# zixunh/vipe

Measured on AMD Instinct MI355X. Metric: dense-BA+flow update iters/s, 512x384 48-KF graph, higher is better.
Workload: dtype f16 (correlation, GRU; fp32 accumulate) + f32 geometry/BA (fp64 reduced system)

## Files before the change

include/vipe_amd.h:

```cpp
#ifndef VIPE_AMD_H
#define VIPE_AMD_H

#include <stdint.h>

#ifdef __cplusplus
extern "C" {
#endif

#define VIPE_F16 0
#define VIPE_F32 1
#define VIPE_F64 2
#define VIPE_U8 3

#define VIPE_OK 0
#define VIPE_EINVAL (-1)
#define VIPE_ENOSPACE (-2)
#define VIPE_EUNSUPPORTED (-3)

#define VIPE_PYRAMID_REFERENCE 0
#define VIPE_PYRAMID_BLOCKED 1

#define VIPE_CAM_PINHOLE 0
#define VIPE_CAM_MEI 1
#define VIPE_CAM_PANORAMA 2
// ... 200 lines not shown

int vipe_corr_sampler_forward(const void* d_in1, const void* d_in2, void* d_out, int B, int C, int H, int W, int kH,
                              int kW, int patchH, int patchW, int padH, int padW, int dilH, int dilW,
                              int dil_patchH, int dil_patchW, int dH, int dW, int dtype, void* stream);
int vipe_corr_sampler_backward(const void* d_in1, const void* d_in2, const void* d_grad_out, void* d_grad1,
                               void* d_grad2, int B, int C, int H, int W, int kH, int kW, int patchH, int patchW,
                               int padH, int padW, int dilH, int dilW, int dil_patchH, int dil_patchW, int dH,
                               int dW, int dtype, void* stream);

int vipe_corr_sampler_forward_host(const float* h_in1, const float* h_in2, float* h_out, int B, int C, int H, int W, int kH,
                                   int kW, int patchH, int patchW, int padH, int padW, int dilH, int dilW, int dil_patchH,
                                   int dil_patchW, int dH, int dW);
int vipe_corr_sampler_backward_host(const float* h_in1, const float* h_in2, const float* h_grad_out, float* h_grad1,
                                    float* h_grad2, int B, int C, int H, int W, int kH, int kW, int patchH, int patchW,
                                    int padH, int padW, int dilH, int dilW, int dil_patchH, int dil_patchW, int dH, int dW);

int vipe_nearest_neighbours(const float* d_query, int qdim, const float* d_tree, int tdim, int64_t M, int64_t N, int knn,
                            float* d_dist, int* d_idx, void* stream);

int vipe_ms_deform_attn_forward(const void* d_value, const int64_t* d_spatial_shapes, const int64_t* d_level_start_index,
                                const void* d_sampling_loc, const void* d_attn_weight, void* d_output, int64_t bs,
                                int64_t Lv, int heads, int C, int L, int64_t Lq, int P, int dtype, void* stream);
int vipe_ms_deform_attn_backward(const void* d_value, const int64_t* d_spatial_shapes, const int64_t* d_level_start_index,
                                 const void* d_sampling_loc, const void* d_attn_weight, const void* d_grad_output,
                                 void* d_grad_value, void* d_grad_sampling_loc, void* d_grad_attn_weight, int64_t bs,
                                 int64_t Lv, int heads, int C, int L, int64_t Lq, int P, int dtype, void* stream);

#define VIPE_ACT_NONE 0
#define VIPE_ACT_RELU 1
#define VIPE_ACT_SIGMOID 2
#define VIPE_ACT_TANH 3
int vipe_conv_pack_weights(const void* d_w_oihw, void* d_w_packed, int Cout, int Cin, int KH, int KW, int src_dtype,
                           void* stream);
int vipe_conv2d_nhwc_f16(const void* d_x, const void* d_w_packed, const float* d_bias, const float* d_extra,
                         void* d_y, int B, int H, int W, int Cin, int cin_total, int cin_off, int Cout,
                         int cout_total, int cout_off, int KH, int KW, int act, void* stream);

int vipe_conv_packed_dims(int Cout, int Cin, int KH, int KW, int* cout_pad, int* cin_pad, int* k_pad);

#define VIPE_CONV_PARTIAL 6
#define VIPE_CONV_HEADS_FUSED 7
#define VIPE_CONV_ACCINIT_F32 0x100
int vipe_conv2d_fused(const void* d_x0, int x0_ctot, int x0_coff, const void* d_x1, int x1_ctot, int x1_coff,
                      int split, const void* d_w_packed, const float* d_bias, const float* d_extra, int extra_stride,
                      int extra_off, void* d_y, int y_ctot, int y_coff, void* d_y2, int y2_ctot, int y2_coff,
                      const void* d_net, int net_ctot, int net_coff, const void* d_z, float* d_fout,
                      const void* d_accinit, int ai_ctot, int ai_coff, int B, int H, int W, int Cin, int Cout, int KH,
                      int KW, int act, int mode, void* stream);

int vipe_heads_fused_ok(int H, int W);
int vipe_heads_border_floats(int E, int H, int W, int64_t* n_floats);
int vipe_heads_finish(float* d_dw, const float* d_border, const float* d_bias, int E, int H, int W, void* stream);

typedef struct {
  const void *corr0_w, *corr2_w, *flow0_w, *flow2_w, *gw_w, *zr_w, *q_w, *zr_s_w, *q_s_w, *heads0_w, *heads2_w, *agg2_w, *eta_w;
  const void *zr_n_w, *zr_x_w;
  const float *corr0_b, *corr2_b, *flow0_b, *flow2_b, *gw_b, *zr_b, *q_b, *heads0_b, *heads2_b, *agg2_b, *eta_b;
  const float* glo_wT;
  const float* glo_b;
  const void *agg1_w, *heads_dw_w;
  const float *agg1_b, *heads_dw_b;
  const void* heads2_frag;
} vipe_update_weights;
typedef struct {
  int E, H, W, n_src;
  const void* levels[4];
  const float* coords;
  const int* slots;
  int h2, w2, pyramid_layout;
  const void* corr;
  const void* motn;
  const void* net;
  void* net_out;
  void* xbuf;
  const void* pgate;
  void *c1, *f1, *zb, *rnet;
  void* hbuf;
  float* dw;
  float *glo, *extra;
  const int *order, *rowptr;
  void *agg, *a2;
  float* eta;
  void* side_stream;
  float* pzr;
  int gate_state;
  float* hborder;
} vipe_update_buffers;
int vipe_update_operator(const vipe_update_weights* weights, const vipe_update_buffers* buffers, void* stream);

int vipe_update_gate_state(const vipe_update_weights* weights, const vipe_update_buffers* buffers, const void* d_net,
                           int parts, void* stream);
typedef struct {
  const vipe_update_weights* weights;
  const vipe_update_buffers* buffers;
  const void* net;
  const int* bounds;
  int n_bounds;
} vipe_gate_state_job;
int vipe_update_gate_state_piece(void* user, int piece, int n_pieces, void* stream);

int vipe_glo_context(const float* d_glo_sum, const float* d_wT, const float* d_bias, float* d_extra, int E, int hw,
                     void* stream);

typedef struct {
  const void* src;
  void* dst;
// ... 88 lines not shown
```

vipe_amd/csrc/conv_mfma.hip:

```cpp
#include <stdlib.h>

#include <type_traits>

#include "common.cuh"

namespace {

typedef _Float16 half8 __attribute__((ext_vector_type(8)));
typedef _Float16 half4 __attribute__((ext_vector_type(4)));
typedef float float16v __attribute__((ext_vector_type(16)));
typedef float float4v __attribute__((ext_vector_type(4)));

enum Epi { EPI_PLAIN = 0, EPI_GLO = 1, EPI_ZR = 2, EPI_Q = 3, EPI_HEADS = 4, EPI_ETA = 5, EPI_PARTIAL = 6, EPI_HEADS_FUSED = 7 };

struct ConvArgs {
  const half_t* x0; int x0_ctot, x0_coff;
  const half_t* x1; int x1_ctot, x1_coff;
  int split;
  const half_t* w;
  const float* bias;
  const float* extra;
  int extra_stride, extra_off;
  half_t* y; int y_ctot, y_coff;
  int B, H, W, Cin, Cin_pad, Cout, Cout_pad, KH, KW, nsteps;
// ... 1051 lines not shown
    for (int j = 0; j < 4; ++j) acc[i][j] = float4v{0.0f, 0.0f, 0.0f, 0.0f};
#pragma unroll
  for (int st = 0; st < 7; ++st) {
    half8 wf[4];
#pragma unroll
    for (int i = 0; i < 4; ++i)
      wf[i] = *reinterpret_cast<const half8*>(lds + (st >> 1) * 16384 + swz(wm * 64 + i * 16 + l16, (st & 1) * 4 + lk));
    const int t0 = min(st * 8 + lk * 2, 48), t1 = min(st * 8 + lk * 2 + 1, 48);
    const int wrow = FLAT ? wn * HALO_TW : wn * C7_PW;
    const int o0 = (wrow + (t0 / 7) * pitch + l16 + t0 % 7) * 8, o1 = (wrow + (t1 / 7) * pitch + l16 + t1 % 7) * 8;
#pragma unroll
    for (int j = 0; j < 4; ++j) {
      const half4 lo = *reinterpret_cast<const half4*>(ldsX + o0 + j * 128);
      const half4 hi = *reinterpret_cast<const half4*>(ldsX + o1 + j * 128);
      const half8 xf = {lo[0], lo[1], lo[2], lo[3], hi[0], hi[1], hi[2], hi[3]};
#pragma unroll
      for (int i = 0; i < 4; ++i) acc[i][j] = __builtin_amdgcn_mfma_f32_16x16x32_f16(wf[i], xf, acc[i][j], 0, 0, 0);
    }
  }
  __syncthreads();
  constexpr int PITCH = 136;
  half_t* stage = reinterpret_cast<half_t*>(lds);
#pragma unroll
  for (int i = 0; i < 4; ++i) {
    const int cl = wm * 64 + i * 16 + 4 * lk;
    const float4 b = *reinterpret_cast<const float4*>(a.bias + cout0 + cl);
#pragma unroll
    for (int j = 0; j < 4; ++j) {
      half4 h;
      h[0] = (half_t)act_apply(acc[i][j][0] + b.x, a.act);
      h[1] = (half_t)act_apply(acc[i][j][1] + b.y, a.act);
      h[2] = (half_t)act_apply(acc[i][j][2] + b.z, a.act);
      h[3] = (half_t)act_apply(acc[i][j][3] + b.w, a.act);
      *reinterpret_cast<half4*>(stage + (wn * 64 + j * 16 + l16) * PITCH + cl) = h;
    }
  }
  __syncthreads();
  const int ch = (tid & 15) * 8, co = cout0 + ch;
#pragma unroll
  for (int it = 0; it < 8; ++it) {
    const int pl = (tid >> 4) + 32 * it;
    const int64_t m = pix_of(pl);
    if (FLAT && m < 0) continue;
    const half8 o = *reinterpret_cast<const half8*>(stage + pl * PITCH + ch);
    half_t* dst = a.y + m * a.y_ctot + a.y_coff + co;
    if (co + 8 <= a.Cout) {
      *reinterpret_cast<half8*>(dst) = o;
    } else {
      for (int q = 0; q < 8 && co + q < a.Cout; ++q) dst[q] = o[q];
    }
  }
}

__global__ void pack_weights_kernel(const void* __restrict__ src, half_t* __restrict__ dst, int Cout, int Cin, int KH,
                                    int KW, int Cout_pad, int Cin_pad, int K_pad, int src_f32, int smallcin) {
  const int64_t total = (int64_t)K_pad * Cout_pad;
  for (int64_t i = (int64_t)blockIdx.x * blockDim.x + threadIdx.x; i < total; i += (int64_t)gridDim.x * blockDim.x) {
    const int kin = (int)(i % 64);
    const int co = (int)((i / 64) % Cout_pad);
    const int s = (int)(i / (64 * (int64_t)Cout_pad));
    const int k = s * 64 + kin;
    int tap, c;
    if (smallcin) { tap = k / 4; c = k % 4; }
    else { tap = k / Cin_pad; c = k % Cin_pad; }
    float v = 0.0f;
    if (co < Cout && c < Cin && tap < KH * KW) {
      const int64_t o = (((int64_t)co * Cin + c) * KH + tap / KW) * KW + tap % KW;
      v = src_f32 ? reinterpret_cast<const float*>(src)[o] : (float)reinterpret_cast<const half_t*>(src)[o];
    }
    dst[i] = (half_t)v;
  }
}

inline int round_up(int x, int m) { return (x + m - 1) / m * m; }

}


extern "C" {

VIPE_EXPORT int vipe_conv_packed_dims(int Cout, int Cin, int KH, int KW, int* cout_pad, int* cin_pad, int* k_pad) {
  if (Cout <= 0 || Cin <= 0 || KH <= 0 || KW <= 0) return VIPE_EINVAL;
  const int cp = Cout <= 32 ? 32 : (Cout <= 64 ? 64 : round_up(Cout, 128));
  int cinp, kp;
  if (Cin == 4) { cinp = 4; kp = round_up(KH * KW * 4, 64); }
  else { cinp = round_up(Cin, 64); kp = KH * KW * cinp; }
  if (cout_pad) *cout_pad = cp;
  if (cin_pad) *cin_pad = cinp;
  if (k_pad) *k_pad = kp;
  return VIPE_OK;
}

VIPE_EXPORT int vipe_conv_pack_weights(const void* d_w_oihw, void* d_w_packed, int Cout, int Cin, int KH, int KW,
                                       int src_dtype, void* stream) {
  VIPE_CHECK_ARG(d_w_oihw && d_w_packed);
  VIPE_CHECK_ARG(src_dtype == VIPE_F16 || src_dtype == VIPE_F32);
  int cp, cinp, kp;
  if (vipe_conv_packed_dims(Cout, Cin, KH, KW, &cp, &cinp, &kp) != VIPE_OK) return VIPE_EINVAL;
  VIPE_CHECK_ARG(Cin == 4 || Cin % 8 == 0);
  const int64_t total = (int64_t)kp * cp;
  pack_weights_kernel<<<(int)std::min<int64_t>((total + 255) / 256, 4096), 256, 0, as_stream(stream)>>>(
      d_w_oihw, (half_t*)d_w_packed, Cout, Cin, KH, KW, cp, cinp, kp, src_dtype == VIPE_F32, Cin == 4);
  return vipe_launch_status();
}

}
// ... 204 lines not shown
                                  int y_coff, void* d_y2, int y2_ctot, int y2_coff, const void* d_net, int net_ctot,
                                  int net_coff, const void* d_z, float* d_fout, const void* d_accinit, int ai_ctot,
                                  int ai_coff, int B, int H, int W, int Cin, int Cout, int KH, int KW, int act, int mode,
                                  void* stream) {
  VIPE_CHECK_ARG(d_x0 && d_w_packed && d_bias);
  VIPE_CHECK_ARG(!d_accinit || (ai_ctot % 4 == 0 && ai_coff % 4 == 0 && ai_coff + Cout <= ai_ctot));
  VIPE_CHECK_ARG(B >= 0 && H > 0 && W > 0 && Cin > 0 && Cout > 0 && (KH & 1) && (KW & 1));
  if (Cin == 4) {
    VIPE_CHECK_ARG(split >= Cin && x0_ctot % 4 == 0 && x0_coff % 4 == 0);
  } else {
    VIPE_CHECK_ARG(Cin % 8 == 0 && x0_ctot % 8 == 0 && x0_coff % 8 == 0);
    VIPE_CHECK_ARG(split >= Cin || (split % 64 == 0 && d_x1 && x1_ctot % 8 == 0 && x1_coff % 8 == 0));
  }
  const int ai_f32 = (mode & VIPE_CONV_ACCINIT_F32) != 0;
  mode &= ~VIPE_CONV_ACCINIT_F32;
  VIPE_CHECK_ARG(mode >= EPI_PLAIN && mode <= EPI_HEADS_FUSED);
  if (mode == EPI_HEADS_FUSED) {
    VIPE_CHECK_ARG(d_fout && d_net && d_y2 && Cin == 128 && Cout == 256 && KH == 3 && KW == 3 && act == VIPE_ACT_RELU &&
                   !d_extra && !d_accinit && !ai_f32 && split >= Cin);
    if (H % HALO_TH != 0 || W % HALO_TW != 0) return VIPE_EUNSUPPORTED;
  }
  if (mode == EPI_PARTIAL) VIPE_CHECK_ARG(d_fout && y_ctot % 4 == 0 && y_coff % 4 == 0 && y_coff + Cout <= y_ctot && !d_extra);
  if (mode == EPI_PLAIN) VIPE_CHECK_ARG(d_y && y_ctot % 4 == 0 && y_coff % 4 == 0);
  if (mode == EPI_GLO) VIPE_CHECK_ARG(d_net && d_fout);
  if (mode == EPI_ZR) VIPE_CHECK_ARG(d_y && d_y2 && d_net && Cout == 256);
  if (mode == EPI_Q) VIPE_CHECK_ARG(d_y && d_net && d_z && Cout == 128);
  if (mode == EPI_HEADS) VIPE_CHECK_ARG(d_fout && Cout == 4);
  if (mode == EPI_ETA) VIPE_CHECK_ARG(d_fout && Cout == 1);
  ConvArgs a = {};
  a.x0 = (const half_t*)d_x0; a.x0_ctot = x0_ctot; a.x0_coff = x0_coff;
  a.x1 = (const half_t*)(d_x1 ? d_x1 : d_x0); a.x1_ctot = d_x1 ? x1_ctot : x0_ctot; a.x1_coff = d_x1 ? x1_coff : x0_coff;
  a.split = split > Cin ? Cin : split;
  a.w = (const half_t*)d_w_packed; a.bias = d_bias; a.extra = d_extra; a.extra_stride = extra_stride; a.extra_off = extra_off;
  a.y = (half_t*)d_y; a.y_ctot = y_ctot; a.y_coff = y_coff;
  a.y2 = (half_t*)d_y2; a.y2_ctot = y2_ctot; a.y2_coff = y2_coff;
  if (mode == EPI_HEADS_FUSED) {
    a.w2 = (const half_t*)d_net; a.border = (float*)d_y2;
    d_net = nullptr; a.y2 = nullptr;
  }
  a.net = (const half_t*)d_net; a.net_ctot = net_ctot; a.net_coff = net_coff;
  a.zbuf = (const half_t*)d_z; a.fout = d_fout;
  a.accinit = (const half_t*)d_accinit; a.ai_ctot = ai_ctot; a.ai_coff = ai_coff; a.ai_f32 = ai_f32;
  a.B = B; a.H = H; a.W = W; a.Cin = Cin; a.Cout = Cout; a.KH = KH; a.KW = KW;
  a.act = act; a.epi = mode;
  return launch_conv(a, as_stream(stream));
}

VIPE_EXPORT int vipe_heads_fused_ok(int H, int W) {
  const char* v = getenv("VIPE_AMD_FUSED_HEADS");
  const bool enabled = !(v && v[0] == '0');
  return enabled && H > 0 && W > 0 && H % HALO_TH == 0 && W % HALO_TW == 0;
}

VIPE_EXPORT int vipe_heads_border_floats(int E, int H, int W, int64_t* n) {
  VIPE_CHECK_ARG(n && E >= 0 && H > 0 && W > 0 && H % HALO_TH == 0 && W % HALO_TW == 0);
  *n = (int64_t)E * (H / HALO_TH) * (W / HALO_TW) * HB_N * 4;
  return VIPE_OK;
}

VIPE_EXPORT int vipe_heads_finish(float* d_dw, const float* d_border, const float* d_bias, int E, int H, int W, void* stream) {
  VIPE_CHECK_ARG(E >= 0 && H > 0 && W > 0 && H % HALO_TH == 0 && W % HALO_TW == 0);
  if (E == 0) return VIPE_OK;
  VIPE_CHECK_ARG(d_dw && d_border && d_bias);
  const int64_t M = (int64_t)E * H * W;
  heads_finish_kernel<<<(unsigned)((M + 255) / 256), 256, 0, as_stream(stream)>>>(d_dw, d_border, d_bias, M, H, W);
  return vipe_launch_status();
}

}
```

vipe_amd/csrc/update_op.hip:

```cpp
#include "common.cuh"

namespace {

__global__ __launch_bounds__(384) void glo_gemm_kernel(const float* __restrict__ glo, const float* __restrict__ wT ,
                                                       const float* __restrict__ b, float* __restrict__ extra, float inv_hw) {
  __shared__ float g[128];
  const int e = blockIdx.x, t = threadIdx.x;
  if (t < 128) g[t] = glo[(int64_t)e * 128 + t] * inv_hw;
  __syncthreads();
  float acc = b[t];
#pragma unroll 8
  for (int k = 0; k < 128; ++k) acc = __builtin_fmaf(g[k], wT[k * 384 + t], acc);
  extra[(int64_t)e * 384 + t] = acc;
}

__global__ __launch_bounds__(256) void update_finish_kernel(const float* __restrict__ coords1, const float* __restrict__ dw,
                                                            const unsigned char* __restrict__ mask, float* __restrict__ target,
                                                            float* __restrict__ weight, const float* __restrict__ eta,
                                                            const int64_t* __restrict__ du, float* __restrict__ damping,
                                                            int64_t n_px, int64_t n_eta, int P) {
  const int64_t i = (int64_t)blockIdx.x * 256 + threadIdx.x;
  if (i < n_px) {
    const float2 c = reinterpret_cast<const float2*>(coords1)[i];
    const float4 d = reinterpret_cast<const float4*>(dw)[i];
// ... 4 lines not shown
  if (i < n_eta) damping[du[i / P] * P + i % P] = eta[i];
}

}

namespace {
hipEvent_t* operator_events() {
  static thread_local hipEvent_t ev[64][4] = {};
  int d = 0;
  (void)hipGetDevice(&d);
  hipEvent_t* e = ev[d & 63];
  for (int i = 0; i < 4; ++i)
    if (!e[i] && hipEventCreateWithFlags(&e[i], hipEventDisableTiming) != hipSuccess) return nullptr;
  return e;
}
}

extern "C" {

VIPE_EXPORT int vipe_update_operator(const vipe_update_weights* wt, const vipe_update_buffers* b, void* stream) {
  VIPE_CHECK_ARG(wt && b && b->E >= 0 && b->H > 0 && b->W > 0);
  if (b->E == 0) return VIPE_OK;
  const int E = b->E, H = b->H, W = b->W;
  hipStream_t s = as_stream(stream);
  int rc;
#define RUN(call)              \
  do {                         \
    rc = (call);               \
    if (rc != VIPE_OK) return rc; \
  } while (0)
  hipStream_t s2 = (hipStream_t)b->side_stream;
  hipEvent_t* ev = s2 ? operator_events() : nullptr;
  if (s2 && !ev) return VIPE_EINVAL;
  void* const stream2 = s2 ? b->side_stream : stream;
#define FORK(i)                                                                                              \
  do {                                                                                                       \
    if (s2 && (hipEventRecord(ev[i], s) != hipSuccess || hipStreamWaitEvent(s2, ev[i], 0) != hipSuccess)) return VIPE_EINVAL; \
  } while (0)
#define JOIN(i)                                                                                              \
  do {                                                                                                       \
    if (s2 && (hipEventRecord(ev[i], s2) != hipSuccess || hipStreamWaitEvent(s, ev[i], 0) != hipSuccess)) return VIPE_EINVAL; \
  } while (0)
  FORK(0);
  if (b->levels[0]) {
    RUN(vipe_corr_lookup_conv1x1_ex(b->levels, b->coords, wt->corr0_w, wt->corr0_b, b->c1, 128, 0, E, H, W, b->h2, b->w2, 128,
                                    VIPE_ACT_RELU, b->slots, b->pyramid_layout, stream, 0, s2 ? 1 : 0));
  } else {
    VIPE_CHECK_ARG(b->corr);
    RUN(vipe_conv2d_fused(b->corr, 200, 0, nullptr, 0, 0, 200, wt->corr0_w, wt->corr0_b, nullptr, 0, 0, b->c1, 128, 0, nullptr,
                          0, 0, nullptr, 0, 0, nullptr, nullptr, nullptr, 0, 0, E, H, W, 200, 128, 1, 1, VIPE_ACT_RELU, 0, stream));
  }
  RUN(vipe_conv2d_fused(b->c1, 128, 0, nullptr, 0, 0, 128, wt->corr2_w, wt->corr2_b, nullptr, 0, 0, b->xbuf, 320, 128, nullptr,
                        0, 0, nullptr, 0, 0, nullptr, nullptr, nullptr, 0, 0, E, H, W, 128, 128, 3, 3, VIPE_ACT_RELU, 0, stream));
  RUN(vipe_conv2d_fused(b->motn, 4, 0, nullptr, 0, 0, 4, wt->flow0_w, wt->flow0_b, nullptr, 0, 0, b->f1, 128, 0, nullptr, 0, 0,
                        nullptr, 0, 0, nullptr, nullptr, nullptr, 0, 0, E, H, W, 4, 128, 7, 7, VIPE_ACT_RELU, 0, stream2));
  RUN(vipe_conv2d_fused(b->f1, 128, 0, nullptr, 0, 0, 128, wt->flow2_w, wt->flow2_b, nullptr, 0, 0, b->xbuf, 320, 256, nullptr,
                        0, 0, nullptr, 0, 0, nullptr, nullptr, nullptr, 0, 0, E, H, W, 128, 64, 3, 3, VIPE_ACT_RELU, 0, stream2));
  JOIN(1);
  const int Es = b->gate_state;
  const bool staged = Es != 0;
  if (staged) VIPE_CHECK_ARG(Es > 0 && Es <= E && b->pgate && b->pzr && wt->zr_x_w);
  if (!staged) {
    if (hipMemsetAsync(b->glo, 0, sizeof(float) * 128 * (size_t)E, s) != hipSuccess) return VIPE_EINVAL;
    RUN(vipe_conv2d_fused(b->net, 128, 0, nullptr, 0, 0, 128, wt->gw_w, wt->gw_b, nullptr, 0, 0, nullptr, 0, 0, nullptr, 0, 0,
                          b->net, 128, 0, nullptr, b->glo, nullptr, 0, 0, E, H, W, 128, 128, 1, 1, VIPE_ACT_NONE, 1, stream));
    glo_gemm_kernel<<<E, 384, 0, s>>>(b->glo, wt->glo_wT, wt->glo_b, b->extra, 1.0f / (float)(H * W));
  }
  if (staged) {
    RUN(vipe_conv2d_fused(b->xbuf, 320, 128, nullptr, 0, 0, 192, wt->zr_x_w, wt->zr_b, b->extra, 384, 0, b->zb, 128, 0, b->rnet,
                          128, 0, b->net, 128, 0, nullptr, nullptr, b->pzr, 256, 0, Es, H, W, 192, 256, 3, 3, VIPE_ACT_NONE,
                          2 | VIPE_CONV_ACCINIT_F32, stream));
    if (Es < E) {
      const int64_t px = (int64_t)Es * H * W;
      auto h16 = [&](const void* p, int c) { return (const void*)((const char*)p + px * c * 2); };
      RUN(vipe_conv2d_fused(h16(b->net, 128), 128, 0, h16(b->xbuf, 320), 320, 128, 128, wt->zr_s_w, wt->zr_b,
                            b->extra + (int64_t)Es * 384, 384, 0, (void*)h16(b->zb, 128), 128, 0, (void*)h16(b->rnet, 128), 128, 0,
                            h16(b->net, 128), 128, 0, nullptr, nullptr, h16(b->pgate, 384), 384, 0, E - Es, H, W, 320, 256, 3, 3,
                            VIPE_ACT_NONE, 2, stream));
    }
    RUN(vipe_conv2d_fused(b->rnet, 128, 0, b->xbuf, 320, 128, 128, wt->q_s_w, wt->q_b, b->extra, 384, 256, b->net_out, 128, 0,
                          nullptr, 0, 0, b->net, 128, 0, b->zb, nullptr, b->pgate, 384, 256, E, H, W, 320, 128, 3, 3,
                          VIPE_ACT_NONE, 3, stream));
  } else if (b->pgate) {
    RUN(vipe_conv2d_fused(b->net, 128, 0, b->xbuf, 320, 128, 128, wt->zr_s_w, wt->zr_b, b->extra, 384, 0, b->zb, 128, 0, b->rnet,
                          128, 0, b->net, 128, 0, nullptr, nullptr, b->pgate, 384, 0, E, H, W, 320, 256, 3, 3, VIPE_ACT_NONE, 2,
                          stream));
    RUN(vipe_conv2d_fused(b->rnet, 128, 0, b->xbuf, 320, 128, 128, wt->q_s_w, wt->q_b, b->extra, 384, 256, b->net_out, 128, 0,
                          nullptr, 0, 0, b->net, 128, 0, b->zb, nullptr, b->pgate, 384, 256, E, H, W, 320, 128, 3, 3,
                          VIPE_ACT_NONE, 3, stream));
  } else {
    RUN(vipe_conv2d_fused(b->net, 128, 0, b->xbuf, 320, 0, 128, wt->zr_w, wt->zr_b, b->extra, 384, 0, b->zb, 128, 0, b->rnet, 128,
                          0, b->net, 128, 0, nullptr, nullptr, nullptr, 0, 0, E, H, W, 448, 256, 3, 3, VIPE_ACT_NONE, 2, stream));
    RUN(vipe_conv2d_fused(b->rnet, 128, 0, b->xbuf, 320, 0, 128, wt->q_w, wt->q_b, b->extra, 384, 256, b->net_out, 128, 0, nullptr,
                          0, 0, b->net, 128, 0, b->zb, nullptr, nullptr, 0, 0, E, H, W, 448, 128, 3, 3, VIPE_ACT_NONE, 3, stream));
  }
  const bool two_tails = s2 && b->n_src > 0;
  const bool by_consumer = wt->agg1_w && wt->agg1_b && wt->heads_dw_w && wt->heads_dw_b;
  auto heads0 = [&](const void* w, const float* bias, int coff, int cout) -> int {
    return vipe_conv2d_fused(b->net_out, 128, 0, nullptr, 0, 0, 128, w, bias, nullptr, 0, 0, b->hbuf, 384, coff, nullptr, 0, 0,
                             nullptr, 0, 0, nullptr, nullptr, nullptr, 0, 0, E, H, W, 128, cout, 3, 3, VIPE_ACT_RELU, 0, stream);
  };
  auto agg_chain = [&](void* st) -> int {
    if (b->n_src <= 0) return VIPE_OK;
    VIPE_CHECK_ARG(b->order && b->rowptr && b->agg && b->a2 && b->eta);
    RUN(vipe_segment_mean_nhwc_f16(b->hbuf, 384, 256, b->order, b->rowptr, b->agg, b->n_src, (int64_t)H * W, 128, st));
    RUN(vipe_conv2d_fused(b->agg, 128, 0, nullptr, 0, 0, 128, wt->agg2_w, wt->agg2_b, nullptr, 0, 0, b->a2, 128, 0, nullptr, 0, 0,
                          nullptr, 0, 0, nullptr, nullptr, nullptr, 0, 0, b->n_src, H, W, 128, 128, 3, 3, VIPE_ACT_RELU, 0, st));
    return vipe_conv2d_fused(b->a2, 128, 0, nullptr, 0, 0, 128, wt->eta_w, wt->eta_b, nullptr, 0, 0, nullptr, 0, 0, nullptr, 0, 0,
                             nullptr, 0, 0, nullptr, b->eta, nullptr, 0, 0, b->n_src, H, W, 128, 1, 3, 3, VIPE_ACT_NONE, 5, st);
  };
// ... 99 lines not shown
```

vipe_amd/slam/update_engine.py:

```python

import ctypes
import os

import torch

from .._lib import check, lib, parse_struct, ptr, stream_ptr

UpdateWeights = parse_struct("vipe_update_weights")
UpdateBuffers = parse_struct("vipe_update_buffers")
GateStateJob = parse_struct("vipe_gate_state_job")

ACT = {"none": 0, "relu": 1, "sigmoid": 2, "tanh": 3}
EPI = {"plain": 0, "glo": 1, "zr": 2, "q": 3, "heads": 4, "eta": 5, "partial": 6, "heads_fused": 7}
ACCINIT_F32 = 0x100
CORR_CH = 200


class _Packed:

    def __init__(self, w_oihw, bias, device):
        w = w_oihw.detach().to(device=device, dtype=torch.float16).contiguous()
        self.cout, self.cin, self.kh, self.kw = w.shape
        cp, cinp, kp = ctypes.c_int(), ctypes.c_int(), ctypes.c_int()
        check(lib().vipe_conv_packed_dims(self.cout, self.cin, self.kh, self.kw, ctypes.addressof(cp),
# ... 141 lines not shown
        if native:
            b = UpdateBuffers()
            b.H, b.W = H, W
            b.pgate, b.pzr, b.glo, b.extra = pgate.data_ptr(), pzr.data_ptr(), glo.data_ptr(), extra.data_ptr()
            for part, n in ((1, E), (2, Es)):
                if parts & part:
                    b.E = n
                    check(lib().vipe_update_gate_state(ctypes.addressof(self._wdesc), ctypes.addressof(b), ptr(net), part,
                                                       stream_ptr(net)), "update_gate_state")
        else:
            if parts & 1:
                glo.zero_()
                self._conv(self.gw, net, 0, E, H, W, mode="glo", net=net, fout=glo)
                check(lib().vipe_glo_context(ptr(glo), ptr(self.glo_w), ptr(self.glo_b), ptr(extra), E, H * W,
                                             stream_ptr(glo)), "glo_context")
            if parts & 2:
                self._conv(self.zr_n, net, 0, Es, H, W, mode="partial", fout=pzr, accinit=pgate, ai_coff=0)
        return dict(net_ptr=net.data_ptr(), pgate_ptr=pgate.data_ptr(), shape=tuple(net.shape), pzr=pzr, extra=extra,
                    n_staged=Es, gen=self._gate_gen)

    def gate_state_job(self, net, pgate, fractions=None, n_staged=None):
        E_all, H, W, _ = net.shape
        E = E_all if n_staged is None else max(1, min(E_all, int(n_staged)))
        self._gate_gen += 1
        glo = self._buf("glo", (E_all, 128), torch.float32)
        extra = self._buf("extra", (E_all, 384), torch.float32)
        pzr = self._buf("pzr", (E, H, W, 256), torch.float32)
        b = UpdateBuffers()
        b.E, b.H, b.W = E, H, W
        b.pgate, b.pzr, b.glo, b.extra = pgate.data_ptr(), pzr.data_ptr(), glo.data_ptr(), extra.data_ptr()
        job = GateStateJob()
        job.weights, job.buffers, job.net = ctypes.addressof(self._wdesc), ctypes.addressof(b), net.data_ptr()
        bounds = None
        if fractions:
            cum, acc = [0], 0.0
            for f in fractions[:-1]:
                acc += f
                cum.append(min(E, int(round(E * acc / sum(fractions)))))
            cum.append(E)
            bounds = (ctypes.c_int * len(cum))(*cum)
            job.bounds, job.n_bounds = ctypes.addressof(bounds), len(cum)
        fn = ctypes.cast(lib().vipe_update_gate_state_piece, ctypes.c_void_p).value
        gs = dict(net_ptr=net.data_ptr(), pgate_ptr=pgate.data_ptr(), shape=tuple(net.shape), pzr=pzr, extra=extra,
                  n_staged=E, keep=(b, job, bounds), gen=self._gate_gen)
        return gs, (lambda stream: (stream.cuda_stream, fn, ctypes.addressof(job)))

    def gate_state_matches(self, gs, net, pgate):
        return (gs is not None and pgate is not None and gs["net_ptr"] == net.data_ptr() and
                gs["pgate_ptr"] == pgate.data_ptr() and gs["shape"] == tuple(net.shape) and gs.get("gen") == self._gate_gen)

    def fused_heads(self, H, W):
        return self.fused_heads_on and bool(lib().vipe_heads_fused_ok(H, W))

    def _hborder(self, E, H, W):
        n = ctypes.c_int64()
        check(lib().vipe_heads_border_floats(E, H, W, ctypes.addressof(n)), "heads_border_floats")
        return self._buf("hborder", (n.value,), torch.float32)

    def _buf(self, name, shape, dtype=torch.float16):
        t = self._bufs.get(name)
        if t is None or tuple(t.shape) != tuple(shape) or t.dtype != dtype:
            t = torch.empty(shape, dtype=dtype, device=self.device)
            self._bufs[name] = t
        return t

    @torch.no_grad()
    def forward_nhwc(self, net, xbuf, corr, motn, ix=None, n_src=None, net_out=None, want_upmask=False, csr=None,
                     pgate=None, native=True, gate_state=None):
        E, H, W, _ = net.shape
        if not self.gate_state_matches(gate_state, net, pgate):
            gate_state = None
        if gate_state is None:
            self._gate_gen += 1
        c1 = self._buf("c1", (E, H, W, 128))
        f1 = self._buf("f1", (E, H, W, 128))
        zb = self._buf("z", (E, H, W, 128))
        rnet = self._buf("rnet", (E, H, W, 128))
        hbuf = self._buf("h", (E, H, W, 384))
        dw = self._buf("dw", (E, H, W, 4), torch.float32)
        glo = self._buf("glo", (E, 128), torch.float32)
        if net_out is None:
            net_out = torch.empty_like(net)
        if native:
            return self._forward_native(net, xbuf, corr, motn, ix, n_src, net_out, want_upmask, csr, pgate,
                                        (c1, f1, zb, rnet, hbuf, dw, glo), gate_state)
        if isinstance(corr, tuple):
            from ..ext import droid_net_ext
            droid_net_ext.corr_lookup_conv1x1(corr[1], corr[2], self.corr0.packed, self.corr0.bias, c1, act="relu",
                                              slots=corr[3] if len(corr) > 3 else None,
                                              grid=corr[4] if len(corr) > 4 else None)
        else:
            self._conv(self.corr0, corr, 0, E, H, W, y=c1, act="relu", cin=CORR_CH)
        self._conv(self.corr2, c1, 0, E, H, W, y=xbuf, y_coff=128, act="relu")
        self._conv(self.flow0, motn, 0, E, H, W, y=f1, act="relu")
        self._conv(self.flow2, f1, 0, E, H, W, y=xbuf, y_coff=256, act="relu")
        extra = self._buf("extra", (E, 384), torch.float32)
        if gate_state is None:
            glo.zero_()
            self._conv(self.gw, net, 0, E, H, W, mode="glo", net=net, fout=glo)
            check(lib().vipe_glo_context(ptr(glo), ptr(self.glo_w), ptr(self.glo_b), ptr(extra), E, H * W, stream_ptr(glo)),
                  "glo_context")
        if gate_state is not None:
            Es = gate_state["n_staged"]
            self._conv(self.zr_x, xbuf, 128, Es, H, W, y=zb, y2=rnet, net=net, mode="zr", extra=extra,
                       accinit=gate_state["pzr"], ai_coff=0, cin=192)
            if Es < E:
                self._conv(self.zr_s, net[Es:], 0, E - Es, H, W, x1=xbuf[Es:], x1_coff=128, split=128, y=zb[Es:], y2=rnet[Es:],
                           net=net[Es:], mode="zr", extra=extra[Es:], accinit=pgate[Es:], ai_coff=0)
            self._conv(self.q_s, rnet, 0, E, H, W, x1=xbuf, x1_coff=128, split=128, y=net_out, net=net, z=zb, mode="q",
                       extra=extra, extra_off=256, accinit=pgate, ai_coff=256)
        elif pgate is not None:
            self._conv(self.zr_s, net, 0, E, H, W, x1=xbuf, x1_coff=128, split=128, y=zb, y2=rnet, net=net, mode="zr",
                       extra=extra, accinit=pgate, ai_coff=0)
            self._conv(self.q_s, rnet, 0, E, H, W, x1=xbuf, x1_coff=128, split=128, y=net_out, net=net, z=zb, mode="q",
                       extra=extra, extra_off=256, accinit=pgate, ai_coff=256)
        else:
            self._conv(self.zr, net, 0, E, H, W, x1=xbuf, split=128, y=zb, y2=rnet, net=net, mode="zr", extra=extra)
            self._conv(self.q, rnet, 0, E, H, W, x1=xbuf, split=128, y=net_out, net=net, z=zb, mode="q", extra=extra,
                       extra_off=256)
        if n_src is None and ix is not None:
            n_src = int(ix.max().item()) + 1 if ix.numel() else 0
        eta = upmask = a2 = None

        def agg_chain():
            order, rowptr = csr if csr is not None else segment_csr(ix, n_src)
            agg = self._buf("agg", (n_src, H, W, 128))
            check(lib().vipe_segment_mean_nhwc_f16(ptr(hbuf), 384, 256, ptr(order), ptr(rowptr), ptr(agg), n_src, H * W,
                                                   128, stream_ptr(hbuf)), "segment_mean")
            a2 = self._buf("a2", (n_src, H, W, 128))
            eta = self._buf("eta", (n_src, H, W), torch.float32)
            self._conv(self.agg2, agg, 0, n_src, H, W, y=a2, act="relu")
            self._conv(self.eta, a2, 0, n_src, H, W, mode="eta", fout=eta)
            return a2, eta

        chain = ix is not None and n_src > 0
        if self.heads_by_consumer and chain and E >= self.op_side_min_edges:
            self._conv(self.agg1, net_out, 0, E, H, W, y=hbuf, y_coff=256, act="relu")
            a2, eta = agg_chain()
            if self.fused_heads(H, W):
                hborder = self._hborder(E, H, W)
                self._conv(self.heads_dw, net_out, 0, E, H, W, act="relu", mode="heads_fused", net=self.heads2_frag,
                           y2=hborder, fout=dw)
                check(lib().vipe_heads_finish(ptr(dw), ptr(hborder), ptr(self.heads2.bias), E, H, W, stream_ptr(dw)),
                      "heads_finish")
            else:
                self._conv(self.heads_dw, net_out, 0, E, H, W, y=hbuf, act="relu")
                self._conv(self.heads2, hbuf, 0, E, H, W, mode="heads", fout=dw, cin=256)
        else:
# ... 101 lines not shown
```

Measured before the change: 279.6.

## Fuse flow encoder 7x7 and 3x3 convolutions into one halo-tiled MFMA kernel

Adds a kernel that computes the 7x7 flow0 conv over a halo tile of the motion input in LDS, applies bias and ReLU, and feeds the result directly into the 3x3 flow2 conv. Output goes straight into xbuf. This removes the round trip of the 128-channel f1 intermediate through global memory and one kernel launch. In exchange it recomputes flow0 on the halo pixels, and it adds a complex pipelined DMA schedule with hand-placed waitcnts. The path is on by default and can be disabled with an environment variable.

```diff
diff --git a/include/vipe_amd.h b/include/vipe_amd.h
--- a/include/vipe_amd.h
+++ b/include/vipe_amd.h
@@ -276,6 +276,11 @@
 int vipe_heads_border_floats(int E, int H, int W, int64_t* n_floats);
 int vipe_heads_finish(float* d_dw, const float* d_border, const float* d_bias, int E, int H, int W, void* stream);
 
+int vipe_flow_fused_ok(int H, int W);
+int vipe_flow_encoder_fused(const void* d_motn, int motn_ctot, int motn_coff, const void* d_w7_packed, const float* d_b7,
+                            const void* d_w3_packed, const float* d_b3, void* d_y, int y_ctot, int y_coff, int E, int H, int W,
+                            void* stream);
+
 typedef struct {
   const void *corr0_w, *corr2_w, *flow0_w, *flow2_w, *gw_w, *zr_w, *q_w, *zr_s_w, *q_s_w, *heads0_w, *heads2_w, *agg2_w, *eta_w;
   const void *zr_n_w, *zr_x_w;
diff --git a/vipe_amd/csrc/conv_mfma.hip b/vipe_amd/csrc/conv_mfma.hip
--- a/vipe_amd/csrc/conv_mfma.hip
+++ b/vipe_amd/csrc/conv_mfma.hip
@@ -1127,6 +1127,194 @@
   }
 }
 
+constexpr int FE_MW = HALO_TW + 8, FE_MH = HALO_TH + 8;
+constexpr int FE_WSTAGE = 64 * 64;
+constexpr int FE_W7BYTES = 4 * 32 * 128;
+constexpr int FE_OFF_X = 3 * FE_WSTAGE, FE_OFF_SINK = FE_OFF_X + H32_XBYTES, FE_OFF_W7 = FE_OFF_SINK + 1024;
+constexpr int FE_OFF_M = FE_OFF_W7 + FE_W7BYTES;
+constexpr int FE_LDS = FE_OFF_M + FE_MW * FE_MH * 8;
+static_assert(FE_LDS <= 76 * 1024 && FE_LDS >= 256 * 72 * 2, "beside a half-CU lookup workgroup; holds the staged tile");
+
+struct FlowEncArgs {
+  const half_t* motn; int m_ctot, m_coff;
+  const half_t* w7; const float* b7;
+  const half_t* w3; const float* b3;
+  half_t* y; int y_ctot, y_coff;
+  int H, W;
+};
+
+__global__ __launch_bounds__(512) __attribute__((amdgpu_waves_per_eu(4, 4))) void flow_encoder_fused_kernel(FlowEncArgs a) {
+  constexpr int MI = 2, NJ = 4, WSTAGE = FE_WSTAGE, CS32 = 4, CS64 = 2, C3 = 64;
+  extern __shared__ __align__(16) unsigned char lds[];
+  const int tid = threadIdx.x, lane = tid & 63, wave = __builtin_amdgcn_readfirstlane(tid >> 6);
+  const int wm = wave >> 2, wn = wave & 3;
+  const int tile = xcd_remap(blockIdx.x, gridDim.x);
+  const int xsegs = a.W / HALO_TW, tiles_per_img = (a.H / HALO_TH) * xsegs;
+  const int e = tile / tiles_per_img, trem = tile % tiles_per_img;
+  const int y0 = (trem / xsegs) * HALO_TH, x0 = (trem % xsegs) * HALO_TW;
+  const int r16 = lane >> 2, sl = lane & 3, l16 = lane & 15, lk = lane >> 4;
+
+  const unsigned ldsW_a = lds_address(lds);
+  const unsigned char* ldsW = lds;
+  unsigned char* ldsX = lds + FE_OFF_X;
+  const unsigned char* ldsW7 = lds + FE_OFF_W7;
+  unsigned char* ldsM = lds + FE_OFF_M;
+  const uint64_t zp64 = uniform64((uint64_t)g_zero_page);
+  const unsigned sink_u = __builtin_amdgcn_readfirstlane(ldsW_a + FE_OFF_SINK);
+
+  const bool wreal = wave < C3 / 16;
+  const int wrow = (wave & 3) * 16 + r16;
+  const unsigned woff = (unsigned)(wrow * 64 + ((sl ^ swzf(wrow)) << 3)) * 2u;
+  const unsigned wdst_u = __builtin_amdgcn_readfirstlane(ldsW_a + (wave & 3) * 1024);
+  const uint64_t wbase = uniform64((uint64_t)a.w3);
+  constexpr unsigned tstride = CS64 * C3 * BK * 2u;
+  auto issueW3 = [&](int tap, int c, int slot, bool more_) {
+    const unsigned off = (unsigned)tap * tstride + ((unsigned)(c >> 1) * C3 * BK + (unsigned)(c & 1) * H32_BK) * 2u;
+    const bool on = more_ && wreal;
+    dma16s(on ? wbase + off : zp64, on ? woff : 0u, on ? wdst_u + slot * WSTAGE : sink_u);
+  };
+  const int r8 = lane >> 3, s8 = lane & 7;
+  const unsigned w7dst_u = __builtin_amdgcn_readfirstlane(ldsW_a + FE_OFF_W7 + wave * 2048);
+  auto issueW7 = [&](int c, int q, bool on) {
+    const int pce = wave * 2 + q, blk = pce >> 2, lr = (pce & 3) * 8 + r8;
+    const uint64_t src = (uint64_t)(a.w7 + ((int64_t)blk * 128 + c * 32 + lr) * 64 + ((s8 ^ ((lr >> 1) & 7)) << 3));
+    dma16v(on ? src : zp64, on ? w7dst_u + q * 1024 : sink_u);
+  };
+
+  issueW7(0, 0, true);
+  issueW7(0, 1, true);
+  issueW3(0, 0, 0, true);
+  issueW3(1, 0, 1, true);
+  for (int i = tid; i < FE_MW * FE_MH; i += 512) {
+    const int hy = i / FE_MW, hx = i % FE_MW;
+    const int y = y0 + hy - 4, x = x0 + hx - 4;
+    uint2 v = make_uint2(0u, 0u);
+    if (y >= 0 && y < a.H && x >= 0 && x < a.W)
+      v = *reinterpret_cast<const uint2*>(a.motn + ((int64_t)(e * a.H + y) * a.W + x) * a.m_ctot + a.m_coff);
+    *reinterpret_cast<uint2*>(ldsM + i * 8) = v;
+  }
+  asm volatile("s_waitcnt vmcnt(0)" ::: "memory");
+  __syncthreads();
+
+  float4v acc16[MI][NJ];
+#pragma unroll
+  for (int i = 0; i < MI; ++i)
+#pragma unroll
+    for (int j = 0; j < NJ; ++j) acc16[i][j] = float4v{0.0f, 0.0f, 0.0f, 0.0f};
+
+  const int wa0 = swz32(wm * MI * 16 + l16, lk);
+  const int Rl0 = wn * HALO_PITCH + l16;
+  const int cb = wave & 1, gq = wave >> 1;
+
+  for (int c = 0; c < CS32; ++c) {
+    const bool more = c + 1 < CS32;
+    {
+      constexpr int NG = 7;
+      const float4 b = *reinterpret_cast<const float4*>(a.b7 + c * 32 + cb * 16 + 4 * lk);
+      float4v acc7[NG];
+      int mb[NG];
+#pragma unroll
+      for (int i = 0; i < NG; ++i) {
+        acc7[i] = float4v{0.0f, 0.0f, 0.0f, 0.0f};
+        const int p = min((gq + 4 * i) * 16 + l16, HALO_ROWS - 1);
+        const int hy = p / HALO_PITCH, hx = p - hy * HALO_PITCH;
+        mb[i] = (hy * FE_MW + hx) * 8;
+      }
+#pragma unroll 1
+      for (int st = 0; st < 7; ++st) {
+        const half8 wf = *reinterpret_cast<const half8*>(ldsW7 + (st >> 1) * 4096 + swz(cb * 16 + l16, (st & 1) * 4 + lk));
+        const int t0 = min(st * 8 + lk * 2, 48), t1 = min(st * 8 + lk * 2 + 1, 48);
+        const int o0 = ((t0 / 7) * FE_MW + t0 % 7) * 8, o1 = ((t1 / 7) * FE_MW + t1 % 7) * 8;
+#pragma unroll
+        for (int i = 0; i < NG; ++i) {
+          if (i == NG - 1 && gq != 0) continue;
+          const half4 lo = *reinterpret_cast<const half4*>(ldsM + mb[i] + o0);
+          const half4 hi = *reinterpret_cast<const half4*>(ldsM + mb[i] + o1);
+          const half8 xf = {lo[0], lo[1], lo[2], lo[3], hi[0], hi[1], hi[2], hi[3]};
+          acc7[i] = __builtin_amdgcn_mfma_f32_16x16x32_f16(wf, xf, acc7[i], 0, 0, 0);
+        }
+      }
+#pragma unroll
+      for (int i = 0; i < NG; ++i) {
+        if (i == NG - 1 && gq != 0) continue;
+        const int p = (gq + 4 * i) * 16 + l16;
+        const int hy = p / HALO_PITCH, hx = p - hy * HALO_PITCH;
+        const int y = y0 + hy - 1, x = x0 + hx - 1;
+        const bool ok = p < HALO_ROWS && y >= 0 && y < a.H && x >= 0 && x < a.W;
+        half4 h;
+        h[0] = ok ? (half_t)fmaxf(acc7[i][0] + b.x, 0.0f) : (half_t)0.0f;
+        h[1] = ok ? (half_t)fmaxf(acc7[i][1] + b.y, 0.0f) : (half_t)0.0f;
+        h[2] = ok ? (half_t)fmaxf(acc7[i][2] + b.z, 0.0f) : (half_t)0.0f;
+        h[3] = ok ? (half_t)fmaxf(acc7[i][3] + b.w, 0.0f) : (half_t)0.0f;
+        *reinterpret_cast<half4*>(ldsX + swz32(p, cb * 2 + (lk >> 1)) + (lk & 1) * 8) = h;
+      }
+    }
+    __syncthreads();
+    {
+      int Rl = Rl0;
+      asm volatile("" : "+v"(Rl));
+      auto tap_step = [&](auto TAPC) {
+        constexpr int TAP = decltype(TAPC)::value;
+        constexpr int T2 = TAP + 2;
+        half8 wf[MI], xf[NJ];
+        const unsigned char* bw = ldsW + (TAP % 3) * WSTAGE;
+        const int xa0 = swz32(Rl + (TAP / 3) * HALO_PITCH + TAP % 3, lk);
+#pragma unroll
+        for (int i = 0; i < MI; ++i) wf[i] = *reinterpret_cast<const half8*>(bw + (wa0 + i * 1024));
+#pragma unroll
+        for (int j = 0; j < NJ; ++j) xf[j] = *reinterpret_cast<const half8*>(ldsX + (xa0 + j * 1024));
+        if constexpr (T2 < 9) issueW3(T2, c, T2 % 3, true);
+        else issueW3(T2 - 9, c + 1, T2 % 3, more);
+        if constexpr (TAP < 2) issueW7(c + 1, TAP, more);
+#pragma unroll
+        for (int j = 0; j < NJ; ++j)
+#pragma unroll
+          for (int i = 0; i < MI; ++i) acc16[i][j] = __builtin_amdgcn_mfma_f32_16x16x32_f16(wf[i], xf[j], acc16[i][j], 0, 0, 0);
+        if constexpr (TAP == 1) asm volatile("s_waitcnt vmcnt(3)" ::: "memory");
+        else if constexpr (TAP == 0 || TAP == 2) asm volatile("s_waitcnt vmcnt(2)" ::: "memory");
+        else asm volatile("s_waitcnt vmcnt(1)" ::: "memory");
+        __syncthreads();
+      };
+      tap_step(std::integral_constant<int, 0>{});
+      tap_step(std::integral_constant<int, 1>{});
+      tap_step(std::integral_constant<int, 2>{});
+      tap_step(std::integral_constant<int, 3>{});
+      tap_step(std::integral_constant<int, 4>{});
+      tap_step(std::integral_constant<int, 5>{});
+      tap_step(std::integral_constant<int, 6>{});
+      tap_step(std::integral_constant<int, 7>{});
+      tap_step(std::integral_constant<int, 8>{});
+    }
+  }
+  asm volatile("s_waitcnt vmcnt(0)" ::: "memory");
+  __syncthreads();
+
+  constexpr int PITCH = C3 + 8;
+  half_t* stage = reinterpret_cast<half_t*>(lds);
+#pragma unroll
+  for (int i = 0; i < MI; ++i) {
+    const int cl = wm * (MI * 16) + i * 16 + 4 * lk;
+    const float4 b = *reinterpret_cast<const float4*>(a.b3 + cl);
+#pragma unroll
+    for (int j = 0; j < NJ; ++j) {
+      half4 h;
+      h[0] = (half_t)fmaxf(acc16[i][j][0] + b.x, 0.0f);
+      h[1] = (half_t)fmaxf(acc16[i][j][1] + b.y, 0.0f);
+      h[2] = (half_t)fmaxf(acc16[i][j][2] + b.z, 0.0f);
+      h[3] = (half_t)fmaxf(acc16[i][j][3] + b.w, 0.0f);
+      *reinterpret_cast<half4*>(stage + (wn * 64 + j * 16 + l16) * PITCH + cl) = h;
+    }
+  }
+  __syncthreads();
+  const int ch = (tid & 7) * 8;
+#pragma unroll
+  for (int it = 0; it < 4; ++it) {
+    const int pl = (tid >> 3) + 64 * it;
+    const int64_t m = ((int64_t)(e * a.H + y0 + (pl >> 6))) * a.W + x0 + (pl & 63);
+    *reinterpret_cast<half8*>(a.y + m * a.y_ctot + a.y_coff + ch) = *reinterpret_cast<const half8*>(stage + pl * PITCH + ch);
+  }
+}
+
 __global__ void pack_weights_kernel(const void* __restrict__ src, half_t* __restrict__ dst, int Cout, int Cin, int KH,
                                     int KW, int Cout_pad, int Cin_pad, int K_pad, int src_f32, int smallcin) {
   const int64_t total = (int64_t)K_pad * Cout_pad;
@@ -1437,6 +1625,32 @@
   return enabled && H > 0 && W > 0 && H % HALO_TH == 0 && W % HALO_TW == 0;
 }
 
+VIPE_EXPORT int vipe_flow_fused_ok(int H, int W) {
+  const char* v = getenv("VIPE_AMD_FUSED_FLOW");
+  const bool enabled = !(v && v[0] == '0');
+  return enabled && H > 0 && W > 0 && H % HALO_TH == 0 && W % HALO_TW == 0;
+}
+
+VIPE_EXPORT int vipe_flow_encoder_fused(const void* d_motn, int motn_ctot, int motn_coff, const void* d_w7_packed,
+                                        const float* d_b7, const void* d_w3_packed, const float* d_b3, void* d_y, int y_ctot,
+                                        int y_coff, int E, int H, int W, void* stream) {
+  VIPE_CHECK_ARG(E >= 0 && H > 0 && W > 0);
+  VIPE_CHECK_ARG(motn_ctot >= 4 && motn_ctot % 4 == 0 && motn_coff >= 0 && motn_coff % 4 == 0 && motn_coff + 4 <= motn_ctot);
+  VIPE_CHECK_ARG(y_ctot % 8 == 0 && y_coff >= 0 && y_coff % 8 == 0 && y_coff + 64 <= y_ctot);
+  if (H % HALO_TH != 0 || W % HALO_TW != 0 || (int64_t)E * H * W >= (1ll << 31)) return VIPE_EUNSUPPORTED;
+  if (E == 0) return VIPE_OK;
+  VIPE_CHECK_ARG(d_motn && d_w7_packed && d_b7 && d_w3_packed && d_b3 && d_y);
+  FlowEncArgs a = {};
+  a.motn = (const half_t*)d_motn; a.m_ctot = motn_ctot; a.m_coff = motn_coff;
+  a.w7 = (const half_t*)d_w7_packed; a.b7 = d_b7; a.w3 = (const half_t*)d_w3_packed; a.b3 = d_b3;
+  a.y = (half_t*)d_y; a.y_ctot = y_ctot; a.y_coff = y_coff; a.H = H; a.W = W;
+  static std::atomic<uint64_t> seen{0};
+  allow_lds(flow_encoder_fused_kernel, seen, FE_LDS);
+  const int tiles = (int)((int64_t)E * H * W / (HALO_TH * HALO_TW));
+  flow_encoder_fused_kernel<<<dim3(tiles), 512, FE_LDS, as_stream(stream)>>>(a);
+  return vipe_launch_status();
+}
+
 VIPE_EXPORT int vipe_heads_border_floats(int E, int H, int W, int64_t* n) {
   VIPE_CHECK_ARG(n && E >= 0 && H > 0 && W > 0 && H % HALO_TH == 0 && W % HALO_TW == 0);
   *n = (int64_t)E * (H / HALO_TH) * (W / HALO_TW) * HB_N * 4;
diff --git a/vipe_amd/csrc/update_op.hip b/vipe_amd/csrc/update_op.hip
--- a/vipe_amd/csrc/update_op.hip
+++ b/vipe_amd/csrc/update_op.hip
@@ -80,10 +80,15 @@
   }
   RUN(vipe_conv2d_fused(b->c1, 128, 0, nullptr, 0, 0, 128, wt->corr2_w, wt->corr2_b, nullptr, 0, 0, b->xbuf, 320, 128, nullptr,
                         0, 0, nullptr, 0, 0, nullptr, nullptr, nullptr, 0, 0, E, H, W, 128, 128, 3, 3, VIPE_ACT_RELU, 0, stream));
-  RUN(vipe_conv2d_fused(b->motn, 4, 0, nullptr, 0, 0, 4, wt->flow0_w, wt->flow0_b, nullptr, 0, 0, b->f1, 128, 0, nullptr, 0, 0,
-                        nullptr, 0, 0, nullptr, nullptr, nullptr, 0, 0, E, H, W, 4, 128, 7, 7, VIPE_ACT_RELU, 0, stream2));
-  RUN(vipe_conv2d_fused(b->f1, 128, 0, nullptr, 0, 0, 128, wt->flow2_w, wt->flow2_b, nullptr, 0, 0, b->xbuf, 320, 256, nullptr,
-                        0, 0, nullptr, 0, 0, nullptr, nullptr, nullptr, 0, 0, E, H, W, 128, 64, 3, 3, VIPE_ACT_RELU, 0, stream2));
+  if (vipe_flow_fused_ok(H, W)) {
+    RUN(vipe_flow_encoder_fused(b->motn, 4, 0, wt->flow0_w, wt->flow0_b, wt->flow2_w, wt->flow2_b, b->xbuf, 320, 256, E, H, W,
+                                stream2));
+  } else {
+    RUN(vipe_conv2d_fused(b->motn, 4, 0, nullptr, 0, 0, 4, wt->flow0_w, wt->flow0_b, nullptr, 0, 0, b->f1, 128, 0, nullptr, 0, 0,
+                          nullptr, 0, 0, nullptr, nullptr, nullptr, 0, 0, E, H, W, 4, 128, 7, 7, VIPE_ACT_RELU, 0, stream2));
+    RUN(vipe_conv2d_fused(b->f1, 128, 0, nullptr, 0, 0, 128, wt->flow2_w, wt->flow2_b, nullptr, 0, 0, b->xbuf, 320, 256, nullptr,
+                          0, 0, nullptr, 0, 0, nullptr, nullptr, nullptr, 0, 0, E, H, W, 128, 64, 3, 3, VIPE_ACT_RELU, 0, stream2));
+  }
   JOIN(1);
   const int Es = b->gate_state;
   const bool staged = Es != 0;
diff --git a/vipe_amd/slam/update_engine.py b/vipe_amd/slam/update_engine.py
--- a/vipe_amd/slam/update_engine.py
+++ b/vipe_amd/slam/update_engine.py
@@ -217,6 +217,9 @@
     def fused_heads(self, H, W):
         return self.fused_heads_on and bool(lib().vipe_heads_fused_ok(H, W))
 
+    def fused_flow(self, H, W):
+        return bool(lib().vipe_flow_fused_ok(H, W))
+
     def _hborder(self, E, H, W):
         n = ctypes.c_int64()
         check(lib().vipe_heads_border_floats(E, H, W, ctypes.addressof(n)), "heads_border_floats")
@@ -257,8 +260,13 @@
         else:
             self._conv(self.corr0, corr, 0, E, H, W, y=c1, act="relu", cin=CORR_CH)
         self._conv(self.corr2, c1, 0, E, H, W, y=xbuf, y_coff=128, act="relu")
-        self._conv(self.flow0, motn, 0, E, H, W, y=f1, act="relu")
-        self._conv(self.flow2, f1, 0, E, H, W, y=xbuf, y_coff=256, act="relu")
+        if self.fused_flow(H, W):
+            check(lib().vipe_flow_encoder_fused(ptr(motn), 4, 0, ptr(self.flow0.packed), ptr(self.flow0.bias),
+                                                ptr(self.flow2.packed), ptr(self.flow2.bias), ptr(xbuf), 320, 256, E, H, W,
+                                                stream_ptr(xbuf)), "flow_encoder_fused")
+        else:
+            self._conv(self.flow0, motn, 0, E, H, W, y=f1, act="relu")
+            self._conv(self.flow2, f1, 0, E, H, W, y=xbuf, y_coff=256, act="relu")
         extra = self._buf("extra", (E, 384), torch.float32)
         if gate_state is None:
             glo.zero_()
```

Result: no change. 279.1 (-0.2%).
